# shiyao-li/NextBestPath

Hardware: AMD Instinct MI355X
Metric: exploration steps/s (+ NBP maps/s) at 256x256 (higher is better)
Workload: dtype f32

## Files before the change

### nextbestpath_amd/csrc/nbp_sim.hip

```cpp
#include "common.h"
#include "nbp_carve.h"
#include "nbp_camera.h"
#pragma clang fp contract(off)

namespace {

__device__ __forceinline__ void shade_pixel(const float* __restrict__ verts, const int* __restrict__ faces,
                                            const float* __restrict__ vcolors, const Cam& cam, int fi, int row, int col, int H,
                                            int W, float tanh_fov, float ambient, float* rgb3) {
    float v[3][3];
    const int i0 = faces[3 * (size_t)fi], i1 = faces[3 * (size_t)fi + 1], i2 = faces[3 * (size_t)fi + 2];
    to_view(verts + 3 * (size_t)i0, cam.R, cam.T, v[0]);
    to_view(verts + 3 * (size_t)i1, cam.R, cam.T, v[1]);
    to_view(verts + 3 * (size_t)i2, cam.R, cam.T, v[2]);
    float e1[3], e2[3], q[3];
#pragma unroll
    for (int c = 0; c < 3; ++c) { e1[c] = v[1][c] - v[0][c]; e2[c] = v[2][c] - v[0][c]; }
    q[0] = e1[1] * v[0][2] - e1[2] * v[0][1];
    q[1] = e1[2] * v[0][0] - e1[0] * v[0][2];
    q[2] = e1[0] * v[0][1] - e1[1] * v[0][0];
    const int s = H < W ? H : W;
    const float dx = pixel_centre_ndc(W, s, col) * tanh_fov;
    const float dy = pixel_centre_ndc(H, s, row) * tanh_fov;
    const float a0 = e1[2] * e2[1] - e1[1] * e2[2], a1 = e1[0] * e2[2] - e1[2] * e2[0], a2 = e1[1] * e2[0] - e1[0] * e2[1];
    const float u0 = v[0][1] * e2[2] - v[0][2] * e2[1], u1 = v[0][2] * e2[0] - v[0][0] * e2[2], u2 = v[0][0] * e2[1] - v[0][1] * e2[0];
    const float inv = 1.f / ((a0 * dx + a1 * dy) + a2);
    const float u = ((u0 * dx + u1 * dy) + u2) * inv;
    const float vv = ((dx * q[0] + dy * q[1]) + q[2]) * inv;
    const float w0 = (1.f - u) - vv;
    const float* c0 = vcolors + 3 * (size_t)i0;
    const float* c1 = vcolors + 3 * (size_t)i1;
    const float* c2 = vcolors + 3 * (size_t)i2;
#pragma unroll
    for (int k = 0; k < 3; ++k) rgb3[k] = ambient * ((w0 * c0[k] + u * c1[k]) + vv * c2[k]);
}


constexpr int COMPACT_CHUNK = 2048;

__device__ __forceinline__ bool pixel_valid(const float* d, const unsigned char* mk, int p, float fov_range) {
    const float z = d[p];
    return (mk ? mk[p] != 0 : z > -1.f) && z < fov_range;
}

__global__ __launch_bounds__(256) void unproject_count_kernel(const float* __restrict__ depth,
                                                              const unsigned char* __restrict__ mask, int HW, int nblk,
                                                              float fov_range, int* __restrict__ blk_count) {
    __shared__ int tot;
    const int f = blockIdx.y, b = blockIdx.x;
    const float* d = depth + (size_t)f * HW;
    const unsigned char* mk = mask ? mask + (size_t)f * HW : nullptr;
    if (threadIdx.x == 0) tot = 0;
    __syncthreads();
    int c = 0;
    for (int p = b * COMPACT_CHUNK + threadIdx.x; p < min((b + 1) * COMPACT_CHUNK, HW); p += 256)
// ... 232 lines not shown
}
__global__ __launch_bounds__(256) void unproject_compact4_kernel(const float* __restrict__ depth, const unsigned char* __restrict__ mask,
                                                                 int HW, int nblk, float fov_range, double gather,
                                                                 const int* __restrict__ blk_count, unsigned* __restrict__ list,
                                                                 int* __restrict__ counts) {
    unproject_compact4_body(blockIdx.x, blockIdx.y, gridDim.x, gridDim.y, depth, mask, HW, nblk, fov_range, gather, blk_count, list, counts);
}
__global__ __launch_bounds__(256) void unproject_compact4_batch_kernel(UnprojBatch b, int HW, int nblk, float fov_range, double gather) {
    const UnprojItem& a = b.it[blockIdx.z];
    unproject_compact4_body(blockIdx.x, blockIdx.y, gridDim.x, gridDim.y, a.depth[blockIdx.y] - (size_t)blockIdx.y * HW, nullptr, HW, nblk,
                            fov_range, gather, a.blk_count, b.list(blockIdx.z), a.counts);
}
template <bool COLOUR>
__global__ __launch_bounds__(256) void unproject_append_kernel(const float* __restrict__ depth, CamSet cams, int H, int W, float tanh_fov,
                                                               unsigned seed, const unsigned* __restrict__ list,
                                                               const int* __restrict__ counts, float* __restrict__ cloud,
                                                               long long* __restrict__ cloud_count, long long capacity, int n_frames,
                                                               int* __restrict__ done_ticket, const float* __restrict__ rgb,
                                                               float* __restrict__ cloud_rgb, const unsigned long long* __restrict__ zface,
                                                               const float* __restrict__ verts, const int* __restrict__ faces,
                                                               const float* __restrict__ vcolors, float ambient, int fence, BinFile bf) {
    unproject_append_body<COLOUR>(blockIdx.x, blockIdx.y, gridDim.x, gridDim.y, depth, cams.c, H, W, tanh_fov, seed, list, counts, cloud, cloud_count,
                          capacity, n_frames, done_ticket, rgb, cloud_rgb, zface, verts, faces, vcolors, ambient, fence, bf);
}
template <bool COLOUR>
__global__ __launch_bounds__(256) void unproject_append_batch_kernel(UnprojBatch b, int H, int W, float tanh_fov, int n_frames, float ambient,
                                                                     int fence) {
    const UnprojItem& a = b.it[blockIdx.z];
    const size_t shift = (size_t)blockIdx.y * H * W;
    unproject_append_body<COLOUR>(blockIdx.x, blockIdx.y, gridDim.x, gridDim.y, a.depth[blockIdx.y] - shift, a.cam, H, W, tanh_fov, a.seed,
                          b.list(blockIdx.z), a.counts, a.cloud, a.cloud_count, a.capacity, n_frames, b.ticket(blockIdx.z), nullptr, a.cloud_rgb,
                          a.zface[blockIdx.y] ? a.zface[blockIdx.y] - shift : nullptr, a.verts, a.faces, a.vcolors, ambient, fence);
}

__global__ void cloud_count_update_kernel(const int* __restrict__ counts, int F, long long* __restrict__ cloud_count,
                                          long long capacity) {
    if (blockIdx.x == 0 && threadIdx.x == 0) {
        long long n = *cloud_count;
        for (int f = 0; f < F; ++f) n += counts[2 * f + 1];
        *cloud_count = n < capacity ? n : capacity;
    }
}

constexpr int TILE = 8;
struct FaceRec { float a[3], un[3], q[3], tnum, pad[2]; };

constexpr int COARSE = 8;
constexpr int SEG_DEFAULT = 16384;
constexpr int HITS = 320;
constexpr unsigned ZBUF_EMPTY = 0x7F7F7F7Fu;

struct BinEntry { int face; unsigned box; };

__device__ __forceinline__ void raster_setup_body(unsigned bx, unsigned by, unsigned gx, unsigned gy, const float* __restrict__ verts, const int* __restrict__ faces,
                                                           int n_faces, const Cam* cams, int H, int W,
                                                           float tanh_fov, float zclip, FaceRec* __restrict__ recs,
                                                           int ctiles_x, int ctiles_y, int* __restrict__ ccount,
                                                           BinEntry* __restrict__ clist, unsigned* __restrict__ zbuf_bits,
                                                           unsigned long long* __restrict__ zface) {
    const int fr = by;
    const int fi = bx * blockDim.x + threadIdx.x;
    if (zface) for (int p = fi; p < H * W; p += gx * blockDim.x) zface[(size_t)fr * H * W + p] = ~0ull;
    else for (int p = fi; p < H * W; p += gx * blockDim.x) zbuf_bits[(size_t)fr * H * W + p] = ZBUF_EMPTY;
    bool have = false;
    int tx0 = 0, tx1 = 0, ty0 = 0, ty1 = 0;
    if (fi < n_faces) {
        const Cam cam = cams[fr];
        float v[3][3];
#pragma unroll
        for (int k = 0; k < 3; ++k) to_view(verts + 3 * (size_t)faces[3 * (size_t)fi + k], cam.R, cam.T, v[k]);
        if (!(v[0][2] <= zclip && v[1][2] <= zclip && v[2][2] <= zclip)) {
            FaceRec r;
            float e1[3], e2[3];
            const float* v0 = v[0];
#pragma unroll
            for (int c = 0; c < 3; ++c) { e1[c] = v[1][c] - v[0][c]; e2[c] = v[2][c] - v[0][c]; }
            r.q[0] = e1[1] * v0[2] - e1[2] * v0[1];
            r.q[1] = e1[2] * v0[0] - e1[0] * v0[2];
            r.q[2] = e1[0] * v0[1] - e1[1] * v0[0];
            r.tnum = (e2[0] * r.q[0] + e2[1] * r.q[1]) + e2[2] * r.q[2];
            r.a[0] = e1[2] * e2[1] - e1[1] * e2[2]; r.a[1] = e1[0] * e2[2] - e1[2] * e2[0]; r.a[2] = e1[1] * e2[0] - e1[0] * e2[1];
            r.un[0] = v0[1] * e2[2] - v0[2] * e2[1]; r.un[1] = v0[2] * e2[0] - v0[0] * e2[2]; r.un[2] = v0[0] * e2[1] - v0[1] * e2[0];
            r.pad[0] = r.pad[1] = 0.f;
            const int s = H < W ? H : W;
            float cmin = 1e30f, cmax = -1e30f, rmin = 1e30f, rmax = -1e30f;
            auto emit = [&](float x, float y, float z) {
                const float nx = x / (z * tanh_fov), ny = y / (z * tanh_fov);
                const float col = ((float)W - (float)s * nx - 1.f) * 0.5f;
                const float row = ((float)H - (float)s * ny - 1.f) * 0.5f;
                cmin = fminf(cmin, col); cmax = fmaxf(cmax, col); rmin = fminf(rmin, row); rmax = fmaxf(rmax, row);
            };
#pragma unroll
            for (int k = 0; k < 3; ++k) {
                const float* a = v[k];
                const float* b = v[(k + 1) % 3];
                const bool ain = a[2] >= zclip, bin_ = b[2] >= zclip;
                if (ain) emit(a[0], a[1], a[2]);
                if (ain != bin_) {
                    const float t = (zclip - a[2]) / (b[2] - a[2]);
                    emit(a[0] + t * (b[0] - a[0]), a[1] + t * (b[1] - a[1]), zclip);
                }
            }
            if (cmax >= cmin) {
                int c0 = (int)floorf(fmaxf(cmin, -1e8f)) - 1, c1 = (int)ceilf(fminf(cmax, 1e8f)) + 1;
                int r0 = (int)floorf(fmaxf(rmin, -1e8f)) - 1, r1 = (int)ceilf(fminf(rmax, 1e8f)) + 1;
                c0 = max(c0, 0); r0 = max(r0, 0); c1 = min(c1, W - 1); r1 = min(r1, H - 1);
                if (c0 <= c1 && r0 <= r1) {
                    recs[(size_t)fr * n_faces + fi] = r;
                    have = true;
                    tx0 = c0 / TILE; tx1 = c1 / TILE; ty0 = r0 / TILE; ty1 = r1 / TILE;
                }
            }
        }
    }
    const int lane = threadIdx.x & 63;
    const unsigned long long lt = (1ull << lane) - 1ull;
    const BinEntry e = {fi, (unsigned)tx0 | ((unsigned)tx1 << 8) | ((unsigned)ty0 << 16) | ((unsigned)ty1 << 24)};
    const int nct = ctiles_x * ctiles_y;
    for (int c0 = 0; c0 < nct; c0 += 64) {
        const int npass = min(64, nct - c0);
        int my_cnt = 0;
        for (int c = 0; c < npass; ++c) {
            const int cx = (c0 + c) % ctiles_x, cy = (c0 + c) / ctiles_x;
            const bool hit = have && tx0 <= cx * COARSE + COARSE - 1 && tx1 >= cx * COARSE && ty0 <= cy * COARSE + COARSE - 1 &&
                             ty1 >= cy * COARSE;
            const int n = __popcll(__ballot(hit));
            if (lane == c) my_cnt = n;
        }
        int my_base = 0;
        if (my_cnt > 0) my_base = atomicAdd(&ccount[fr * nct + c0 + lane], my_cnt);
        for (int c = 0; c < npass; ++c) {
            const int cx = (c0 + c) % ctiles_x, cy = (c0 + c) / ctiles_x;
            const bool hit = have && tx0 <= cx * COARSE + COARSE - 1 && tx1 >= cx * COARSE && ty0 <= cy * COARSE + COARSE - 1 &&
                             ty1 >= cy * COARSE;
            const unsigned long long bal = __ballot(hit);
            const int base = __shfl(my_base, c);
            if (hit) clist[((size_t)fr * nct + c0 + c) * n_faces + base + __popcll(bal & lt)] = e;
        }
    }
}

constexpr int RB = 2;
__device__ __forceinline__ int ballot_rank(unsigned long long bal) {
    return (int)__builtin_amdgcn_mbcnt_hi((unsigned)(bal >> 32), __builtin_amdgcn_mbcnt_lo((unsigned)bal, 0u));
}
__device__ __forceinline__ void raster_block_body(unsigned bx, unsigned by, const FaceRec* __restrict__ recs, int n_faces, int H, int W,
                                                  float tanh_fov, float zclip, int tiles_x, int tiles_y, int ctiles_x,
                                                  const int* __restrict__ ccount, const BinEntry* __restrict__ clist,
                                                  unsigned* __restrict__ zbuf_bits, unsigned long long* __restrict__ zface, int SEG) {
    __shared__ BinEntry bhits[HITS];
    __shared__ int nb_sh;
    __shared__ __attribute__((aligned(16))) FaceRec sh[4][64];
    __shared__ int shf[4][64];
    const int fr = by;
    const int blocks_x = (tiles_x + RB - 1) / RB, blocks_y = (tiles_y + RB - 1) / RB;
    const int nblocks = blocks_x * blocks_y;
    const int blk = bx % nblocks, seg = bx / nblocks;
    const int bxx = blk % blocks_x, byy = blk / blocks_x;
    const int nct = ctiles_x * ((tiles_y + COARSE - 1) / COARSE);
    const int ct = ((byy * RB) / COARSE) * ctiles_x + (bxx * RB) / COARSE;
    const int n = ccount[fr * nct + ct];
    const int s0 = seg * SEG;
    if (s0 >= n) return;
    const int s1 = min(n, s0 + SEG);
    const int tid = threadIdx.x, lane = tid & 63, wave = __builtin_amdgcn_readfirstlane(tid >> 6);
    const BinEntry* lst = clist + ((size_t)fr * nct + ct) * n_faces;
    const int btx0 = bxx * RB, btx1 = btx0 + RB - 1, bty0 = byy * RB, bty1 = bty0 + RB - 1;
    const int tx = btx0 + (wave & 1), ty = bty0 + (wave >> 1);
    const bool live = tx < tiles_x && ty < tiles_y;
    const int col = tx * TILE + (lane & 7), row = ty * TILE + (lane >> 3);
    const int s = H < W ? H : W;
    const float ndc_x = pixel_centre_ndc(W, s, col);
    const float ndc_y = pixel_centre_ndc(H, s, row);
    const float dx = ndc_x * tanh_fov, dy = ndc_y * tanh_fov;
    const FaceRec* rb = recs + (size_t)fr * n_faces;
    float zbest = 3.0e38f;
    int fbest = -1;
    const float eps = 1e-6f;
    for (int c0 = s0; c0 < s1; c0 += HITS) {
        const int c1 = min(s1, c0 + HITS);
        if (tid == 0) nb_sh = 0;
        __syncthreads();
        for (int base = c0; base < c1; base += 256) {
            bool in = false;
            BinEntry e = {0, 0u};
            if (base + tid < c1) {
                e = lst[base + tid];
                in = btx1 >= (int)(e.box & 255u) && btx0 <= (int)((e.box >> 8) & 255u) && bty1 >= (int)((e.box >> 16) & 255u) &&
                     bty0 <= (int)(e.box >> 24);
            }
            const unsigned long long bal = __ballot(in);
            int wbase = 0;
            if (lane == 0 && bal) wbase = atomicAdd(&nb_sh, __popcll(bal));
            wbase = __shfl(wbase, 0);
            if (in) bhits[wbase + ballot_rank(bal)] = e;
        }
        __syncthreads();
        const int nb = nb_sh;
        if (live)
            for (int hb = 0; hb < nb; hb += 64) {
                bool in = false;
                int face = 0;
                if (hb + lane < nb) {
                    const BinEntry e = bhits[hb + lane];
                    face = e.face;
                    in = tx >= (int)(e.box & 255u) && tx <= (int)((e.box >> 8) & 255u) && ty >= (int)((e.box >> 16) & 255u) &&
                         ty <= (int)(e.box >> 24);
                }
                const unsigned long long bal = __ballot(in);
                const int m = __popcll(bal);
                if (in) {
                    const int k = ballot_rank(bal);
                    sh[wave][k] = rb[face];
                    shf[wave][k] = face;
                }
                __builtin_amdgcn_s_waitcnt(0);
                __builtin_amdgcn_wave_barrier();
                for (int k = 0; k < m; ++k) {
                    const FaceRec& f = sh[wave][k];
                    const float det = (f.a[0] * dx + f.a[1] * dy) + f.a[2];
                    if (fabsf(det) < 1e-12f) continue;
                    const float inv = 1.f / det;
                    const float u = ((f.un[0] * dx + f.un[1] * dy) + f.un[2]) * inv;
                    const float vv = ((dx * f.q[0] + dy * f.q[1]) + f.q[2]) * inv;
                    const float z = f.tnum * inv;
                    if (u >= -eps && vv >= -eps && u + vv <= 1.f + eps && z > zclip) {
                        const int fid = shf[wave][k];
                        if (z < zbest || (z == zbest && fid < fbest)) { zbest = z; fbest = fid; }
                    }
                }
                __builtin_amdgcn_wave_barrier();
            }
        __syncthreads();
    }
    if (live && row < H && col < W && zbest < 1.0e38f) {
        const size_t pix = ((size_t)fr * H + row) * W + col;
        if (zface) atomicMin(&zface[pix], ((unsigned long long)__float_as_uint(zbest) << 32) | (unsigned)fbest);
        else atomicMin(&zbuf_bits[pix], __float_as_uint(zbest));
    }
}

__global__ __launch_bounds__(256) void raster_finalize_kernel(float* __restrict__ zbuf, long long n) {
    for (long long i = (long long)blockIdx.x * blockDim.x + threadIdx.x; i < n; i += (long long)gridDim.x * blockDim.x)
        if (!(zbuf[i] < 1.0e38f)) zbuf[i] = -1.f;
}

__device__ __forceinline__ void raster_shade_body(unsigned bx, unsigned by, unsigned gx, unsigned gy, const unsigned long long* __restrict__ zface,
                                                           const float* __restrict__ verts, const int* __restrict__ faces,
                                                           const float* __restrict__ vcolors, const Cam* cams, int H, int W,
                                                           float tanh_fov, float ambient, float* __restrict__ zbuf_or_null,
                                                           float* __restrict__ rgb_or_null, double* __restrict__ gray_sum) {
    const int fr = by;
    const int p = bx * blockDim.x + threadIdx.x;
    float gray = 0.f;
    if (p < H * W) {
        const size_t pix = (size_t)fr * H * W + p;
        const unsigned long long zf = zface[pix];
        float c[3] = {1.f, 1.f, 1.f};
        if (zbuf_or_null) zbuf_or_null[pix] = zf != ~0ull ? __uint_as_float((unsigned)(zf >> 32)) : -1.f;
        if (rgb_or_null) {
            if (zf != ~0ull) shade_pixel(verts, faces, vcolors, cams[fr], (int)(unsigned)zf, p / W, p % W, H, W, tanh_fov, ambient, c);
            rgb_or_null[3 * pix] = c[0]; rgb_or_null[3 * pix + 1] = c[1]; rgb_or_null[3 * pix + 2] = c[2];
            gray = (0.299f * c[0] + 0.587f * c[1]) + 0.114f * c[2];
        }
    }
    if (!gray_sum) return;
    double gs = (double)gray;
    for (int o = 32; o; o >>= 1) gs += __shfl_xor(gs, o);
    if ((threadIdx.x & 63) == 0) atomicAdd(&gray_sum[fr], gs);
}

struct RasterItem {
    const float* verts; const int* faces; const float* vcolors; FaceRec* recs; int* ccount; BinEntry* clist; float* zbuf;
    unsigned long long* zface; int n_faces; unsigned gx_setup, gx_tile; Cam cam[4];
};
struct RasterBatch { RasterItem it[STEP_BATCH]; };

__global__ __launch_bounds__(256) void raster_setup_kernel(const float* __restrict__ verts, const int* __restrict__ faces, int n_faces,
                                                           CamSet cams, int H, int W, float tanh_fov, float zclip,
                                                           FaceRec* __restrict__ recs, int ctiles_x, int ctiles_y, int* __restrict__ ccount,
                                                           BinEntry* __restrict__ clist, unsigned* __restrict__ zbuf_bits,
                                                           unsigned long long* __restrict__ zface) {
    raster_setup_body(blockIdx.x, blockIdx.y, gridDim.x, gridDim.y, verts, faces, n_faces, cams.c, H, W, tanh_fov, zclip, recs, ctiles_x,
                      ctiles_y, ccount, clist, zbuf_bits, zface);
}
__global__ __launch_bounds__(256) void raster_clear_batch_kernel(RasterBatch b, int n_counters) {
    int* c = b.it[blockIdx.y].ccount;
    for (int i = blockIdx.x * blockDim.x + threadIdx.x; i < n_counters; i += gridDim.x * blockDim.x) c[i] = 0;
}
__global__ __launch_bounds__(256) void raster_setup_batch_kernel(RasterBatch b, int H, int W, float tanh_fov, float zclip, int ctiles_x,
                                                                 int ctiles_y) {
    const RasterItem& a = b.it[blockIdx.z];
    if (blockIdx.x >= a.gx_setup) return;
    raster_setup_body(blockIdx.x, blockIdx.y, a.gx_setup, gridDim.y, a.verts, a.faces, a.n_faces, a.cam, H, W, tanh_fov, zclip, a.recs,
                      ctiles_x, ctiles_y, a.ccount, a.clist, nullptr, a.zface);
}
__global__ __launch_bounds__(256) void raster_tile_kernel(const FaceRec* __restrict__ recs, int n_faces, int H, int W, float tanh_fov,
                                                          float zclip, int tiles_x, int tiles_y, int ctiles_x, int ctiles_y,
                                                          const int* __restrict__ ccount, const BinEntry* __restrict__ clist,
                                                          unsigned* __restrict__ zbuf_bits, unsigned long long* __restrict__ zface, int SEG) {
    raster_block_body(blockIdx.x, blockIdx.y, recs, n_faces, H, W, tanh_fov, zclip, tiles_x, tiles_y, ctiles_x, ccount, clist, zbuf_bits, zface,
                      SEG);
}
__global__ __launch_bounds__(256) void raster_tile_batch_kernel(RasterBatch b, int H, int W, float tanh_fov, float zclip, int tiles_x,
                                                                int tiles_y, int ctiles_x, int ctiles_y, int SEG) {
    const RasterItem& a = b.it[blockIdx.z];
    if (blockIdx.x >= a.gx_tile) return;
    raster_block_body(blockIdx.x, blockIdx.y, a.recs, a.n_faces, H, W, tanh_fov, zclip, tiles_x, tiles_y, ctiles_x, a.ccount, a.clist, nullptr,
                      a.zface, SEG);
}
__global__ __launch_bounds__(256) void raster_shade_kernel(const unsigned long long* __restrict__ zface, const float* __restrict__ verts,
                                                           const int* __restrict__ faces, const float* __restrict__ vcolors, CamSet cams,
                                                           int H, int W, float tanh_fov, float ambient, float* __restrict__ zbuf_or_null,
                                                           float* __restrict__ rgb_or_null, double* __restrict__ gray_sum) {
    raster_shade_body(blockIdx.x, blockIdx.y, gridDim.x, gridDim.y, zface, verts, faces, vcolors, cams.c, H, W, tanh_fov, ambient, zbuf_or_null,
                      rgb_or_null, gray_sum);
}
__global__ __launch_bounds__(256) void raster_depth_batch_kernel(RasterBatch b, int H, int W, float tanh_fov) {
    const RasterItem& a = b.it[blockIdx.z];
    raster_shade_body(blockIdx.x, blockIdx.y, gridDim.x, gridDim.y, a.zface, a.verts, a.faces, a.vcolors, a.cam, H, W, tanh_fov, 0.f, a.zbuf,
                      nullptr, nullptr);
}

__global__ __launch_bounds__(256) void contrast_kernel(float* __restrict__ rgb, int HW3, const double* __restrict__ gray_sum,
                                                       int HW, float factor) {
    const int fr = blockIdx.y;
    const float mean = (float)(gray_sum[fr] / (double)HW);
    for (int i = blockIdx.x * blockDim.x + threadIdx.x; i < HW3; i += gridDim.x * blockDim.x) {
        const float v = factor * rgb[(size_t)fr * HW3 + i] + (1.f - factor) * mean;
        rgb[(size_t)fr * HW3 + i] = fminf(fmaxf(v, 0.f), 1.f);
    }
}

__device__ __forceinline__ float ray_tri(const float* o, const float* d, const float* a, const float* b, const float* c) {
    const float e1[3] = {b[0] - a[0], b[1] - a[1], b[2] - a[2]};
    const float e2[3] = {c[0] - a[0], c[1] - a[1], c[2] - a[2]};
    const float p[3] = {d[1] * e2[2] - d[2] * e2[1], d[2] * e2[0] - d[0] * e2[2], d[0] * e2[1] - d[1] * e2[0]};
    const float det = (e1[0] * p[0] + e1[1] * p[1]) + e1[2] * p[2];
    if (fabsf(det) < 1e-12f) return -1.f;
    const float inv = 1.f / det;
    const float tv[3] = {o[0] - a[0], o[1] - a[1], o[2] - a[2]};
    const float u = ((tv[0] * p[0] + tv[1] * p[1]) + tv[2] * p[2]) * inv;
    if (u < 0.f || u > 1.f) return -1.f;
    const float q[3] = {tv[1] * e1[2] - tv[2] * e1[1], tv[2] * e1[0] - tv[0] * e1[2], tv[0] * e1[1] - tv[1] * e1[0]};
    const float v = ((d[0] * q[0] + d[1] * q[1]) + d[2] * q[2]) * inv;
    if (v < 0.f || u + v > 1.f) return -1.f;
    const float t = ((e2[0] * q[0] + e2[1] * q[1]) + e2[2] * q[2]) * inv;
    return t > 0.f ? t : -1.f;
}

__global__ __launch_bounds__(256) void segments_hit_kernel(const float* __restrict__ verts, const int* __restrict__ faces,
                                                           int n_faces, const float* __restrict__ segs, int* __restrict__ hit) {
    const int e = blockIdx.y;
    const int fi = blockIdx.x * blockDim.x + threadIdx.x;
    if (fi >= n_faces) return;
    const float* sg = segs + 6 * (size_t)e;
    float d[3] = {sg[3] - sg[0], sg[4] - sg[1], sg[5] - sg[2]};
    const float len = sqrtf((d[0] * d[0] + d[1] * d[1]) + d[2] * d[2]);
    if (!(len > 0.f)) return;
    d[0] /= len; d[1] /= len; d[2] /= len;
    const int* f = faces + 3 * (size_t)fi;
    const float t = ray_tri(sg, d, verts + 3 * (size_t)f[0], verts + 3 * (size_t)f[1], verts + 3 * (size_t)f[2]);
// ... 280 lines not shown
                                                 list, counts2);
    if ((rc = nbp_launch_status())) return rc;
    auto append = cloud_rgb_or_null ? unproject_append_kernel<true> : unproject_append_kernel<false>;
    append<<<grid, 256, 0, st>>>(depth, cams, H, W, tan_half_fov, seed, list, counts2, cloud, cloud_count, capacity, n_frames, nullptr,
                                 rgb_or_null, cloud_rgb_or_null, sh.zface, sh.verts, sh.faces, sh.vcolors, sh.ambient, 0,
                                 BinFile{nullptr, nullptr, nullptr, 0});
    if ((rc = nbp_launch_status())) return rc;
    cloud_count_update_kernel<<<1, 64, 0, st>>>(counts2, n_frames, cloud_count, capacity);
    return nbp_launch_status();
}

constexpr size_t RASTER_WS_SLACK = 256;
struct RasterWs { FaceRec* recs; int* ccount; BinEntry* clist; unsigned long long* zface; double* gray; size_t nct; };
static RasterWs raster_ws_layout(Carver& c, int n_faces, int n_frames, int H, int W, bool rgb) {
    const size_t nct = (size_t)nbp_cdiv(nbp_cdiv(W, TILE), COARSE) * nbp_cdiv(nbp_cdiv(H, TILE), COARSE) * n_frames;
    return {c.take<FaceRec>((size_t)n_frames * n_faces), c.take<int>(nct), c.take<BinEntry>(nct * n_faces),
            rgb ? c.take<unsigned long long>((size_t)n_frames * H * W) : nullptr, rgb ? c.take<double>(MAX_CAMS) : nullptr, nct};
}
static size_t raster_ws_bytes(int n_faces, int n_frames, int H, int W, bool rgb) {
    if (n_faces < 1 || n_frames < 1 || H < 1 || W < 1) return 0;
    return carved_bytes(RASTER_WS_SLACK, raster_ws_layout, n_faces, n_frames, H, W, rgb);
}

extern "C" size_t nbp_raster_workspace_bytes(int n_faces, int n_frames, int H, int W, int bin_cap) {
    (void)bin_cap;
    return raster_ws_bytes(n_faces, n_frames, H, W, false);
}

extern "C" size_t nbp_raster_rgb_workspace_bytes(int n_faces, int n_frames, int H, int W) {
    return raster_ws_bytes(n_faces, n_frames, H, W, true);
}

static int raster_launch(const float* verts, int n_verts, const int* faces, int n_faces, const float* cams12_host, int n_frames,
                         int H, int W, float tan_half_fov, float z_clip, float* zbuf, const float* vcolors, float ambient,
                         float contrast, float* rgb, void* ws, size_t ws_bytes, void* stream,
                         unsigned long long* zface_out = nullptr) {
    NBP_RETURN_IF(!verts || !faces || !cams12_host || !zbuf || !ws, NBP_E_ARG);
    NBP_RETURN_IF(n_verts < 3 || n_faces < 1 || n_frames < 1 || n_frames > MAX_CAMS || H < 1 || W < 1, NBP_E_ARG);
    NBP_RETURN_IF(!(z_clip > 0.f), NBP_E_ARG);
    const int tiles_x = (int)nbp_cdiv(W, TILE), tiles_y = (int)nbp_cdiv(H, TILE);
    NBP_RETURN_IF(tiles_x > 256 || tiles_y > 256, NBP_E_SHAPE);
    NBP_RETURN_IF(ws_bytes < raster_ws_bytes(n_faces, n_frames, H, W, rgb != nullptr && !zface_out), NBP_E_WS);
    hipStream_t st = (hipStream_t)stream;
    const int ctiles_x = (int)nbp_cdiv(tiles_x, COARSE), ctiles_y = (int)nbp_cdiv(tiles_y, COARSE);
    const RasterWs L = carve(ws, raster_ws_layout, n_faces, n_frames, H, W, rgb != nullptr && !zface_out);
    FaceRec* const recs = L.recs;
    int* const ccount = L.ccount;
    BinEntry* const clist = L.clist;
    unsigned long long* const zface = zface_out ? zface_out : L.zface;
    double* const gray = L.gray;
    const long long npx = (long long)n_frames * H * W;
    hipError_t e = hipMemsetAsync(ccount, 0, L.nct * sizeof(int), st);
    if (e != hipSuccess) return (int)e;
    dim3 g1((unsigned)nbp_cdiv(n_faces, 256), (unsigned)n_frames);
    raster_setup_kernel<<<g1, 256, 0, st>>>(verts, faces, n_faces, camset_from_host(cams12_host, n_frames), H, W,
                                            tan_half_fov, z_clip, recs, ctiles_x, ctiles_y, ccount, clist, (unsigned*)zbuf, zface);
    int rc = nbp_launch_status();
    if (rc) return rc;
    const bool need_gray = gray && contrast != 1.f;
    if (need_gray) {
        e = hipMemsetAsync(gray, 0, (size_t)n_frames * sizeof(double), st);
        if (e != hipSuccess) return (int)e;
    }
    constexpr int SEG = SEG_DEFAULT;
    const int nseg = (int)nbp_cdiv(n_faces, SEG);
    dim3 g2((unsigned)((int)nbp_cdiv(tiles_x, RB) * (int)nbp_cdiv(tiles_y, RB) * nseg), (unsigned)n_frames);
    raster_tile_kernel<<<g2, 256, 0, st>>>(recs, n_faces, H, W, tan_half_fov, z_clip, tiles_x, tiles_y, ctiles_x, ctiles_y,
                                          ccount, clist, (unsigned*)zbuf, zface, SEG);
    if ((rc = nbp_launch_status())) return rc;
    if (!zface) {
        raster_finalize_kernel<<<nbp_ew_grid(npx, 256), 256, 0, st>>>(zbuf, npx);
        return nbp_launch_status();
    }
    dim3 g3((unsigned)nbp_cdiv((long long)H * W, 256), (unsigned)n_frames);
    raster_shade_kernel<<<g3, 256, 0, st>>>(zface, verts, faces, vcolors, camset_from_host(cams12_host, n_frames), H, W,
                                            tan_half_fov, ambient, zbuf, rgb, need_gray ? gray : nullptr);
    if ((rc = nbp_launch_status())) return rc;
    if (need_gray) {
        dim3 g4((unsigned)nbp_ew_grid((long long)H * W * 3, 256), (unsigned)n_frames);
        contrast_kernel<<<g4, 256, 0, st>>>(rgb, H * W * 3, gray, H * W, contrast);
        rc = nbp_launch_status();
    }
    return rc;
}

extern "C" int nbp_raster_zbuf_f32(const float* verts, int n_verts, const int* faces, int n_faces, const float* cams12_host,
                                   int n_frames, int H, int W, float tan_half_fov, float z_clip, int bin_cap, float* zbuf,
                                   int* overflow_flag, void* ws, size_t ws_bytes, void* stream) {
    NBP_ENTER();
    (void)bin_cap; (void)overflow_flag;
    return raster_launch(verts, n_verts, faces, n_faces, cams12_host, n_frames, H, W, tan_half_fov, z_clip, zbuf, nullptr, 0.f,
                         1.f, nullptr, ws, ws_bytes, stream);
}

extern "C" int nbp_raster_rgbz_f32(const float* verts, int n_verts, const int* faces, int n_faces, const float* vcolors3,
                                   const float* cams12_host, int n_frames, int H, int W, float tan_half_fov, float z_clip,
                                   float ambient, float contrast_factor, float* zbuf, float* rgb, void* ws, size_t ws_bytes,
                                   void* stream) {
    NBP_ENTER();
    NBP_RETURN_IF(!vcolors3 || !rgb, NBP_E_ARG);
    return raster_launch(verts, n_verts, faces, n_faces, cams12_host, n_frames, H, W, tan_half_fov, z_clip, zbuf, vcolors3,
                         ambient, contrast_factor, rgb, ws, ws_bytes, stream);
}

extern "C" int nbp_raster_zface_f32(const float* verts, int n_verts, const int* faces, int n_faces, const float* cams12_host,
                                    int n_frames, int H, int W, float tan_half_fov, float z_clip, float* zbuf, void* zface,
                                    void* ws, size_t ws_bytes, void* stream) {
    NBP_ENTER();
    NBP_RETURN_IF(!zface, NBP_E_ARG);
    return raster_launch(verts, n_verts, faces, n_faces, cams12_host, n_frames, H, W, tan_half_fov, z_clip, zbuf, nullptr, 0.f,
                         1.f, nullptr, ws, ws_bytes, stream, (unsigned long long*)zface);
}

extern "C" int nbp_unproject_append_shaded_batch_f32(int n, const float* const* depth, const void* const* zface, const float* const* verts,
                                                     const int* const* faces, const float* const* vcolors, const float* cams12_host,
                                                     int n_frames, int H, int W, float tan_half_fov, float fov_range,
                                                     double gathering_factor, const unsigned* seeds, float ambient, int* const* counts2,
                                                     float* const* cloud, float* const* cloud_rgb, long long* const* cloud_count,
                                                     const long long* capacity, void* const* ws, size_t ws_bytes_each, void* stream) {
    NBP_ENTER();
    NBP_RETURN_IF(n < 1 || n > STEP_BATCH || !depth || !cams12_host || !seeds || !counts2 || !cloud || !cloud_count || !capacity || !ws, NBP_E_ARG);
    NBP_RETURN_IF(n_frames < 1 || n_frames > 4 || H < 2 || W < 2 || !(gathering_factor >= 0.0 && gathering_factor <= 1.0), NBP_E_ARG);
    NBP_RETURN_IF(ws_bytes_each < nbp_unproject_workspace_bytes(n_frames, H, W), NBP_E_WS);
    const int HW = H * W;
    NBP_RETURN_IF((HW & 3) != 0, NBP_E_SHAPE);
// ... 3 lines not shown
    UnprojBatch b;
    bool any_colour = false;
    for (int r = 0; r < STEP_BATCH; ++r) {
        const int q = r < n ? r : 0;
        NBP_RETURN_IF(!counts2[q] || !cloud[q] || !cloud_count[q] || capacity[q] < 1 || !ws[q], NBP_E_ARG);
        UnprojItem& a = b.it[r];
        const UnprojectWs L = carve(ws[q], unproject_ws_layout, n_frames, H, W);
        a.blk_count = L.blk_count;
        b.ticket_off = (int)(L.ticket - L.blk_count);
        b.list_off_bytes = (unsigned)((char*)L.list - (char*)L.blk_count);
        a.counts = counts2[q]; a.cloud = cloud[q]; a.cloud_count = cloud_count[q]; a.capacity = capacity[q];
        const bool col = zface && zface[(size_t)q * n_frames] && cloud_rgb && cloud_rgb[q] && verts && faces && vcolors;
        a.cloud_rgb = col ? cloud_rgb[q] : nullptr;
        any_colour = any_colour || col;
        for (int f = 0; f < 4; ++f) {
            const int g = f < n_frames ? f : 0;
            a.depth[f] = depth[(size_t)q * n_frames + g];
            NBP_RETURN_IF(!a.depth[f] || ((uintptr_t)a.depth[f] & 15) != 0, NBP_E_ARG);
            a.zface[f] = col ? (const unsigned long long*)zface[(size_t)q * n_frames + g] : nullptr;
        }
        a.verts = col ? verts[q] : nullptr; a.faces = col ? faces[q] : nullptr; a.vcolors = col ? vcolors[q] : nullptr;
        a.seed = seeds[q];
        cams_from_host(cams12_host + (size_t)q * n_frames * 12, n_frames, a.cam, 4);
    }
    dim3 g4((unsigned)nb4, (unsigned)n_frames, (unsigned)n);
    unproject_count4_batch_kernel<<<g4, 256, 0, st>>>(b, HW, nb4, fov_range);
    int rc = nbp_launch_status();
    if (rc) return rc;
    unproject_compact4_batch_kernel<<<g4, 256, 0, st>>>(b, HW, nb4, fov_range, gathering_factor);
    if ((rc = nbp_launch_status())) return rc;
    const int max_keep = (int)((double)H * W * gathering_factor) + 1;
    dim3 grid((unsigned)nbp_cdiv(max_keep, 256), (unsigned)n_frames, (unsigned)n);
    auto append = any_colour ? unproject_append_batch_kernel<true> : unproject_append_batch_kernel<false>;
    append<<<grid, 256, 0, st>>>(b, H, W, tan_half_fov, n_frames, ambient, ticket_fence());
    return nbp_launch_status();
}

extern "C" int nbp_raster_zface_batch_f32(int n, const float* const* verts, const int* n_verts, const int* const* faces, const int* n_faces,
                                          const float* cams12_host, int n_frames, int H, int W, float tan_half_fov, float z_clip,
                                          float* const* zbuf, void* const* zface, void* const* ws, const size_t* ws_bytes, void* stream) {
    NBP_ENTER();
    NBP_RETURN_IF(n < 1 || n > STEP_BATCH || !verts || !n_verts || !faces || !n_faces || !cams12_host || !zbuf || !zface || !ws || !ws_bytes,
                  NBP_E_ARG);
    NBP_RETURN_IF(n_frames < 1 || n_frames > 4 || H < 1 || W < 1, NBP_E_ARG);
    NBP_RETURN_IF(!(z_clip > 0.f), NBP_E_ARG);
    const int tiles_x = (int)nbp_cdiv(W, TILE), tiles_y = (int)nbp_cdiv(H, TILE);
    NBP_RETURN_IF(tiles_x > 256 || tiles_y > 256, NBP_E_SHAPE);
    hipStream_t st = (hipStream_t)stream;
    const int ctiles_x = (int)nbp_cdiv(tiles_x, COARSE), ctiles_y = (int)nbp_cdiv(tiles_y, COARSE);
    const size_t nct = (size_t)ctiles_x * ctiles_y * n_frames;
    constexpr int SEG = SEG_DEFAULT;
    RasterBatch b;
    unsigned g_setup = 1, g_tile = 1;
    for (int r = 0; r < STEP_BATCH; ++r) {
        const int q = r < n ? r : 0;
        NBP_RETURN_IF(!verts[q] || !faces[q] || n_verts[q] < 3 || n_faces[q] < 1 || !zbuf[q] || !zface[q] || !ws[q], NBP_E_ARG);
        NBP_RETURN_IF(ws_bytes[q] < raster_ws_bytes(n_faces[q], n_frames, H, W, false), NBP_E_WS);
        RasterItem& a = b.it[r];
        const RasterWs L = carve(ws[q], raster_ws_layout, n_faces[q], n_frames, H, W, false);
        a.recs = L.recs; a.ccount = L.ccount; a.clist = L.clist;
        a.verts = verts[q]; a.faces = faces[q]; a.vcolors = nullptr; a.zbuf = zbuf[q]; a.zface = (unsigned long long*)zface[q];
        a.n_faces = n_faces[q];
        a.gx_setup = r < n ? (unsigned)nbp_cdiv(n_faces[q], 256) : 0;
        a.gx_tile = r < n ? (unsigned)((int)nbp_cdiv(tiles_x, RB) * (int)nbp_cdiv(tiles_y, RB) * (int)nbp_cdiv(n_faces[q], SEG)) : 0;
        if (a.gx_setup > g_setup) g_setup = a.gx_setup;
        if (a.gx_tile > g_tile) g_tile = a.gx_tile;
        cams_from_host(cams12_host + (size_t)q * n_frames * 12, n_frames, a.cam, 4);
    }
    raster_clear_batch_kernel<<<dim3(1, (unsigned)n), 256, 0, st>>>(b, (int)nct);
    int rc = nbp_launch_status();
    if (rc) return rc;
    raster_setup_batch_kernel<<<dim3(g_setup, (unsigned)n_frames, (unsigned)n), 256, 0, st>>>(b, H, W, tan_half_fov, z_clip, ctiles_x, ctiles_y);
    if ((rc = nbp_launch_status())) return rc;
    raster_tile_batch_kernel<<<dim3(g_tile, (unsigned)n_frames, (unsigned)n), 256, 0, st>>>(b, H, W, tan_half_fov, z_clip, tiles_x, tiles_y,
                                                                                          ctiles_x, ctiles_y, SEG);
    if ((rc = nbp_launch_status())) return rc;
    raster_depth_batch_kernel<<<dim3((unsigned)nbp_cdiv((long long)H * W, 256), (unsigned)n_frames, (unsigned)n), 256, 0, st>>>(b, H, W,
                                                                                                                          tan_half_fov);
    return nbp_launch_status();
}

extern "C" int nbp_shade_image_f32(const void* zface, const float* verts, const int* faces, const float* vcolors3,
                                   const float* cams12_host, int n_frames, int H, int W, float tan_half_fov, float ambient,
                                   float contrast_factor, float* rgb, void* stream) {
    NBP_ENTER();
    NBP_RETURN_IF(!zface || !verts || !faces || !vcolors3 || !cams12_host || !rgb, NBP_E_ARG);
    NBP_RETURN_IF(n_frames < 1 || n_frames > MAX_CAMS || H < 1 || W < 1, NBP_E_ARG);
    NBP_RETURN_IF(contrast_factor != 1.f, NBP_E_SHAPE);
    dim3 g3((unsigned)nbp_cdiv((long long)H * W, 256), (unsigned)n_frames);
    raster_shade_kernel<<<g3, 256, 0, (hipStream_t)stream>>>((const unsigned long long*)zface, verts, faces, vcolors3,
                                                             camset_from_host(cams12_host, n_frames), H, W, tan_half_fov,
                                                             ambient, nullptr, rgb, nullptr);
    return nbp_launch_status();
}

extern "C" int nbp_segments_hit_mesh_f32(const float* verts, const int* faces, int n_faces, const float* segs6, int n_segs,
                                         int* hit, void* stream) {
    NBP_ENTER();
    NBP_RETURN_IF(!verts || !faces || !segs6 || !hit || n_faces < 1 || n_segs < 1 || n_segs > 65535, NBP_E_ARG);
    hipStream_t st = (hipStream_t)stream;
    hipError_t e = hipMemsetAsync(hit, 0, (size_t)n_segs * sizeof(int), st);
    if (e != hipSuccess) return (int)e;
    dim3 g((unsigned)nbp_cdiv(n_faces, 256), (unsigned)n_segs);
    segments_hit_kernel<<<g, 256, 0, st>>>(verts, faces, n_faces, segs6, hit);
    return nbp_launch_status();
}

extern "C" int nbp_axis_ray_counts_f32(const float* verts, const int* faces, int n_faces, const float* pts3, int n_pts,
                                       int* counts3, void* stream) {
    NBP_ENTER();
    NBP_RETURN_IF(!verts || !faces || !pts3 || !counts3 || n_faces < 1 || n_pts < 1 || n_pts > 65535, NBP_E_ARG);
    hipStream_t st = (hipStream_t)stream;
    hipError_t e = hipMemsetAsync(counts3, 0, (size_t)n_pts * 3 * sizeof(int), st);
    if (e != hipSuccess) return (int)e;
    dim3 g((unsigned)nbp_cdiv(n_faces, 256), (unsigned)n_pts);
    axis_ray_count_kernel<<<g, 256, 0, st>>>(verts, faces, n_faces, pts3, counts3);
    return nbp_launch_status();
}

extern "C" int nbp_carve_update_f32(const float* proxy_pts3, int P, const float* depth, const unsigned char* mask_or_null,
                                    const float* cam12_host, int H, int W, float tan_half_fov, float zfar, float fov_range,
                                    float tol, float score_threshold, float* n_inside, float* n_behind, float* occ,
                                    float* out_of_field, void* stream) {
    NBP_ENTER();
    NBP_RETURN_IF(!proxy_pts3 || !depth || !cam12_host || !n_inside || !n_behind || !occ || !out_of_field, NBP_E_ARG);
    NBP_RETURN_IF(P < 1 || H < 2 || W < 2, NBP_E_ARG);
    Cam cam;
    for (int k = 0; k < 9; ++k) cam.R[k] = cam12_host[k];
    for (int k = 0; k < 3; ++k) cam.T[k] = cam12_host[9 + k];
// ... 234 lines not shown
```

Before: 2369.

## Add conservative tile-level face culling and owner-writes path for single-segment rasterization

Adds a conservative interval test that rejects faces which cannot cover any pixel of an 8x8 tile before the per-pixel ray-triangle loop. When the face count fits in one segment, each tile block now owns its pixels: it writes depth and face id directly instead of pre-clearing the buffers, using atomicMin, and running the separate depth/finalize pass. Binning now walks only the wave's bounding rectangle of coarse tiles instead of every coarse tile. Together these cut clears, atomics, a kernel launch and wasted intersection work, at the cost of extra per-face cull arithmetic and more template code paths.

Result: no change. 2389, median of 4 (+0.8%).

```diff
diff --git a/nextbestpath_amd/csrc/nbp_raster_cull.h b/nextbestpath_amd/csrc/nbp_raster_cull.h
--- /dev/null
+++ b/nextbestpath_amd/csrc/nbp_raster_cull.h
@@ -0,0 +1,52 @@
+#pragma once
+#include <math.h>
+
+#if defined(__HIPCC__)
+#define NBP_CULL_HD __host__ __device__ __forceinline__
+#else
+#define NBP_CULL_HD inline
+#endif
+#if defined(__clang__)
+#pragma clang fp contract(off)
+#endif
+#if defined(__HIP_DEVICE_COMPILE__)
+#define NBP_CULL_PHASE() __builtin_amdgcn_sched_barrier(0)
+#else
+#define NBP_CULL_PHASE() ((void)0)
+#endif
+
+constexpr float RASTER_CULL_H8 = 4.76837158203125e-7f;
+constexpr float RASTER_CULL_TINY = 1e-30f;
+constexpr float RASTER_CULL_EPS = 2e-6f;
+
+struct RasterCullRange { float lo, hi, err; };
+
+NBP_CULL_HD RasterCullRange raster_cull_range(float c0, float c1, float c2, float s, float dxa, float dxb, float dya, float dyb) {
+    const float mx = fmaxf(fabsf(dxa), fabsf(dxb)), my = fmaxf(fabsf(dya), fabsf(dyb));
+    const float xa = c0 * dxa, xb = c0 * dxb, ya = c1 * dya, yb = c1 * dyb;
+    const float l0 = s * ((xa + ya) + c2), l1 = s * ((xb + ya) + c2), l2 = s * ((xa + yb) + c2), l3 = s * ((xb + yb) + c2);
+    RasterCullRange r;
+    r.lo = fminf(fminf(l0, l1), fminf(l2, l3));
+    r.hi = fmaxf(fmaxf(l0, l1), fmaxf(l2, l3));
+    r.err = RASTER_CULL_H8 * ((fabsf(c0) * mx + fabsf(c1) * my) + fabsf(c2)) + RASTER_CULL_TINY;
+    return r;
+}
+
+NBP_CULL_HD bool raster_cull_reject(const float* a, const float* un, const float* q, float tnum, float dxa, float dxb, float dya,
+                                    float dyb) {
+    const float s = (a[0] * dxa + a[1] * dya) + a[2] > 0.f ? 1.f : -1.f;
+    const RasterCullRange D = raster_cull_range(a[0], a[1], a[2], s, dxa, dxb, dya, dyb);
+    if (!(D.lo > 2.f * D.err)) return false;
+    if (s * tnum <= 0.f) return true;
+    const float dm = D.hi + 2.f * D.err;
+    NBP_CULL_PHASE();
+    const RasterCullRange U = raster_cull_range(un[0], un[1], un[2], s, dxa, dxb, dya, dyb);
+    if (U.hi < -(RASTER_CULL_EPS * dm + 2.f * U.err)) return true;
+    NBP_CULL_PHASE();
+    const RasterCullRange Q = raster_cull_range(q[0], q[1], q[2], s, dxa, dxb, dya, dyb);
+    if (Q.hi < -(RASTER_CULL_EPS * dm + 2.f * Q.err)) return true;
+    const float lim = (dm + RASTER_CULL_EPS * dm) + 4.f * (U.err + Q.err);
+    NBP_CULL_PHASE();
+    const RasterCullRange W = raster_cull_range(un[0] + q[0], un[1] + q[1], un[2] + q[2], s, dxa, dxb, dya, dyb);
+    return W.lo > lim && W.hi <= 3.0e38f;
+}
diff --git a/nextbestpath_amd/csrc/nbp_sim.hip b/nextbestpath_amd/csrc/nbp_sim.hip
--- a/nextbestpath_amd/csrc/nbp_sim.hip
+++ b/nextbestpath_amd/csrc/nbp_sim.hip
@@ -1,6 +1,7 @@
 #include "common.h"
 #include "nbp_carve.h"
 #include "nbp_camera.h"
+#include "nbp_raster_cull.h"
 #pragma clang fp contract(off)
 
 namespace {
@@ -339,6 +340,7 @@
 
 struct BinEntry { int face; unsigned box; };
 
+template <bool OWN>
 __device__ __forceinline__ void raster_setup_body(unsigned bx, unsigned by, unsigned gx, unsigned gy, const float* __restrict__ verts, const int* __restrict__ faces,
                                                            int n_faces, const Cam* cams, int H, int W,
                                                            float tanh_fov, float zclip, FaceRec* __restrict__ recs,
@@ -347,8 +349,10 @@
                                                            unsigned long long* __restrict__ zface) {
     const int fr = by;
     const int fi = bx * blockDim.x + threadIdx.x;
-    if (zface) for (int p = fi; p < H * W; p += gx * blockDim.x) zface[(size_t)fr * H * W + p] = ~0ull;
-    else for (int p = fi; p < H * W; p += gx * blockDim.x) zbuf_bits[(size_t)fr * H * W + p] = ZBUF_EMPTY;
+    if (!OWN) {
+        if (zface) for (int p = fi; p < H * W; p += gx * blockDim.x) zface[(size_t)fr * H * W + p] = ~0ull;
+        else for (int p = fi; p < H * W; p += gx * blockDim.x) zbuf_bits[(size_t)fr * H * W + p] = ZBUF_EMPTY;
+    }
     bool have = false;
     int tx0 = 0, tx1 = 0, ty0 = 0, ty1 = 0;
     if (fi < n_faces) {
@@ -404,25 +408,37 @@
     const unsigned long long lt = (1ull << lane) - 1ull;
     const BinEntry e = {fi, (unsigned)tx0 | ((unsigned)tx1 << 8) | ((unsigned)ty0 << 16) | ((unsigned)ty1 << 24)};
     const int nct = ctiles_x * ctiles_y;
-    for (int c0 = 0; c0 < nct; c0 += 64) {
-        const int npass = min(64, nct - c0);
+    int rx0 = have ? tx0 / COARSE : 0x7fff, rx1 = have ? tx1 / COARSE : -1, ry0 = have ? ty0 / COARSE : 0x7fff, ry1 = have ? ty1 / COARSE : -1;
+    for (int o = 32; o; o >>= 1) {
+        rx0 = min(rx0, __shfl_xor(rx0, o)); rx1 = max(rx1, __shfl_xor(rx1, o));
+        ry0 = min(ry0, __shfl_xor(ry0, o)); ry1 = max(ry1, __shfl_xor(ry1, o));
+    }
+    rx0 = __builtin_amdgcn_readfirstlane(rx0); rx1 = __builtin_amdgcn_readfirstlane(rx1);
+    ry0 = __builtin_amdgcn_readfirstlane(ry0); ry1 = __builtin_amdgcn_readfirstlane(ry1);
+    if (rx1 < rx0) return;
+    const int rw = rx1 - rx0 + 1, nrect = rw * (ry1 - ry0 + 1);
+    for (int c0 = 0; c0 < nrect; c0 += 64) {
+        const int npass = min(64, nrect - c0);
         int my_cnt = 0;
         for (int c = 0; c < npass; ++c) {
-            const int cx = (c0 + c) % ctiles_x, cy = (c0 + c) / ctiles_x;
+            const int cx = rx0 + (c0 + c) % rw, cy = ry0 + (c0 + c) / rw;
             const bool hit = have && tx0 <= cx * COARSE + COARSE - 1 && tx1 >= cx * COARSE && ty0 <= cy * COARSE + COARSE - 1 &&
                              ty1 >= cy * COARSE;
             const int n = __popcll(__ballot(hit));
             if (lane == c) my_cnt = n;
         }
         int my_base = 0;
-        if (my_cnt > 0) my_base = atomicAdd(&ccount[fr * nct + c0 + lane], my_cnt);
+        if (my_cnt > 0) {
+            const int i = c0 + lane;
+            my_base = atomicAdd(&ccount[fr * nct + (ry0 + i / rw) * ctiles_x + rx0 + i % rw], my_cnt);
+        }
         for (int c = 0; c < npass; ++c) {
-            const int cx = (c0 + c) % ctiles_x, cy = (c0 + c) / ctiles_x;
+            const int cx = rx0 + (c0 + c) % rw, cy = ry0 + (c0 + c) / rw;
             const bool hit = have && tx0 <= cx * COARSE + COARSE - 1 && tx1 >= cx * COARSE && ty0 <= cy * COARSE + COARSE - 1 &&
                              ty1 >= cy * COARSE;
             const unsigned long long bal = __ballot(hit);
             const int base = __shfl(my_base, c);
-            if (hit) clist[((size_t)fr * nct + c0 + c) * n_faces + base + __popcll(bal & lt)] = e;
+            if (hit) clist[((size_t)fr * nct + cy * ctiles_x + cx) * n_faces + base + __popcll(bal & lt)] = e;
         }
     }
 }
@@ -431,6 +447,7 @@
 __device__ __forceinline__ int ballot_rank(unsigned long long bal) {
     return (int)__builtin_amdgcn_mbcnt_hi((unsigned)(bal >> 32), __builtin_amdgcn_mbcnt_lo((unsigned)bal, 0u));
 }
+template <bool OWN>
 __device__ __forceinline__ void raster_block_body(unsigned bx, unsigned by, const FaceRec* __restrict__ recs, int n_faces, int H, int W,
                                                   float tanh_fov, float zclip, int tiles_x, int tiles_y, int ctiles_x,
                                                   const int* __restrict__ ccount, const BinEntry* __restrict__ clist,
@@ -448,7 +465,7 @@
     const int ct = ((byy * RB) / COARSE) * ctiles_x + (bxx * RB) / COARSE;
     const int n = ccount[fr * nct + ct];
     const int s0 = seg * SEG;
-    if (s0 >= n) return;
+    if (!OWN && s0 >= n) return;
     const int s1 = min(n, s0 + SEG);
     const int tid = threadIdx.x, lane = tid & 63, wave = __builtin_amdgcn_readfirstlane(tid >> 6);
     const BinEntry* lst = clist + ((size_t)fr * nct + ct) * n_faces;
@@ -460,6 +477,10 @@
     const float ndc_x = pixel_centre_ndc(W, s, col);
     const float ndc_y = pixel_centre_ndc(H, s, row);
     const float dx = ndc_x * tanh_fov, dy = ndc_y * tanh_fov;
+    const float dxa = __int_as_float(__builtin_amdgcn_readlane(__float_as_int(dx), 0));
+    const float dxb = __int_as_float(__builtin_amdgcn_readlane(__float_as_int(dx), 7));
+    const float dya = __int_as_float(__builtin_amdgcn_readlane(__float_as_int(dy), 0));
+    const float dyb = __int_as_float(__builtin_amdgcn_readlane(__float_as_int(dy), 56));
     const FaceRec* rb = recs + (size_t)fr * n_faces;
     float zbest = 3.0e38f;
     int fbest = -1;
@@ -498,12 +519,22 @@
                 const int m = __popcll(bal);
                 if (in) {
                     const int k = ballot_rank(bal);
-                    sh[wave][k] = rb[face];
+                    const FaceRec& r = rb[face];
+                    FaceRec& d = sh[wave][k];
+#pragma unroll
+                    for (int c = 0; c < 3; ++c) { d.a[c] = r.a[c]; d.un[c] = r.un[c]; d.q[c] = r.q[c]; }
+                    d.tnum = r.tnum;
                     shf[wave][k] = face;
                 }
                 __builtin_amdgcn_s_waitcnt(0);
                 __builtin_amdgcn_wave_barrier();
-                for (int k = 0; k < m; ++k) {
+                bool keep = false;
+                if (lane < m) {
+                    const FaceRec& f = sh[wave][lane];
+                    keep = !raster_cull_reject(f.a, f.un, f.q, f.tnum, dxa, dxb, dya, dyb);
+                }
+                for (unsigned long long todo = __ballot(keep); todo; todo &= todo - 1ull) {
+                    const int k = __builtin_ctzll(todo);
                     const FaceRec& f = sh[wave][k];
                     const float det = (f.a[0] * dx + f.a[1] * dy) + f.a[2];
                     if (fabsf(det) < 1e-12f) continue;
@@ -520,7 +551,14 @@
             }
         __syncthreads();
     }
-    if (live && row < H && col < W && zbest < 1.0e38f) {
+    if (OWN) {
+        if (live && row < H && col < W) {
+            const size_t pix = ((size_t)fr * H + row) * W + col;
+            const bool hit = zbest < 1.0e38f;
+            if (zface) zface[pix] = hit ? ((unsigned long long)__float_as_uint(zbest) << 32) | (unsigned)fbest : ~0ull;
+            if (zbuf_bits) zbuf_bits[pix] = __float_as_uint(hit ? zbest : -1.f);
+        }
+    } else if (live && row < H && col < W && zbest < 1.0e38f) {
         const size_t pix = ((size_t)fr * H + row) * W + col;
         if (zface) atomicMin(&zface[pix], ((unsigned long long)__float_as_uint(zbest) << 32) | (unsigned)fbest);
         else atomicMin(&zbuf_bits[pix], __float_as_uint(zbest));
@@ -563,38 +601,42 @@
 };
 struct RasterBatch { RasterItem it[STEP_BATCH]; };
 
+template <bool OWN>
 __global__ __launch_bounds__(256) void raster_setup_kernel(const float* __restrict__ verts, const int* __restrict__ faces, int n_faces,
                                                            CamSet cams, int H, int W, float tanh_fov, float zclip,
                                                            FaceRec* __restrict__ recs, int ctiles_x, int ctiles_y, int* __restrict__ ccount,
                                                            BinEntry* __restrict__ clist, unsigned* __restrict__ zbuf_bits,
                                                            unsigned long long* __restrict__ zface) {
-    raster_setup_body(blockIdx.x, blockIdx.y, gridDim.x, gridDim.y, verts, faces, n_faces, cams.c, H, W, tanh_fov, zclip, recs, ctiles_x,
+    raster_setup_body<OWN>(blockIdx.x, blockIdx.y, gridDim.x, gridDim.y, verts, faces, n_faces, cams.c, H, W, tanh_fov, zclip, recs, ctiles_x,
                       ctiles_y, ccount, clist, zbuf_bits, zface);
 }
 __global__ __launch_bounds__(256) void raster_clear_batch_kernel(RasterBatch b, int n_counters) {
     int* c = b.it[blockIdx.y].ccount;
     for (int i = blockIdx.x * blockDim.x + threadIdx.x; i < n_counters; i += gridDim.x * blockDim.x) c[i] = 0;
 }
+template <bool OWN>
 __global__ __launch_bounds__(256) void raster_setup_batch_kernel(RasterBatch b, int H, int W, float tanh_fov, float zclip, int ctiles_x,
                                                                  int ctiles_y) {
     const RasterItem& a = b.it[blockIdx.z];
     if (blockIdx.x >= a.gx_setup) return;
-    raster_setup_body(blockIdx.x, blockIdx.y, a.gx_setup, gridDim.y, a.verts, a.faces, a.n_faces, a.cam, H, W, tanh_fov, zclip, a.recs,
+    raster_setup_body<OWN>(blockIdx.x, blockIdx.y, a.gx_setup, gridDim.y, a.verts, a.faces, a.n_faces, a.cam, H, W, tanh_fov, zclip, a.recs,
                       ctiles_x, ctiles_y, a.ccount, a.clist, nullptr, a.zface);
 }
+template <bool OWN>
 __global__ __launch_bounds__(256) void raster_tile_kernel(const FaceRec* __restrict__ recs, int n_faces, int H, int W, float tanh_fov,
                                                           float zclip, int tiles_x, int tiles_y, int ctiles_x, int ctiles_y,
                                                           const int* __restrict__ ccount, const BinEntry* __restrict__ clist,
                                                           unsigned* __restrict__ zbuf_bits, unsigned long long* __restrict__ zface, int SEG) {
-    raster_block_body(blockIdx.x, blockIdx.y, recs, n_faces, H, W, tanh_fov, zclip, tiles_x, tiles_y, ctiles_x, ccount, clist, zbuf_bits, zface,
-                      SEG);
-}
+    raster_block_body<OWN>(blockIdx.x, blockIdx.y, recs, n_faces, H, W, tanh_fov, zclip, tiles_x, tiles_y, ctiles_x, ccount, clist, zbuf_bits,
+                           zface, SEG);
+}
+template <bool OWN>
 __global__ __launch_bounds__(256) void raster_tile_batch_kernel(RasterBatch b, int H, int W, float tanh_fov, float zclip, int tiles_x,
                                                                 int tiles_y, int ctiles_x, int ctiles_y, int SEG) {
     const RasterItem& a = b.it[blockIdx.z];
     if (blockIdx.x >= a.gx_tile) return;
-    raster_block_body(blockIdx.x, blockIdx.y, a.recs, a.n_faces, H, W, tanh_fov, zclip, tiles_x, tiles_y, ctiles_x, a.ccount, a.clist, nullptr,
-                      a.zface, SEG);
+    raster_block_body<OWN>(blockIdx.x, blockIdx.y, a.recs, a.n_faces, H, W, tanh_fov, zclip, tiles_x, tiles_y, ctiles_x, a.ccount, a.clist,
+                           OWN ? (unsigned*)a.zbuf : nullptr, a.zface, SEG);
 }
 __global__ __launch_bounds__(256) void raster_shade_kernel(const unsigned long long* __restrict__ zface, const float* __restrict__ verts,
                                                            const int* __restrict__ faces, const float* __restrict__ vcolors, CamSet cams,
@@ -981,9 +1023,13 @@
     const long long npx = (long long)n_frames * H * W;
     hipError_t e = hipMemsetAsync(ccount, 0, L.nct * sizeof(int), st);
     if (e != hipSuccess) return (int)e;
+    constexpr int SEG = SEG_DEFAULT;
+    const int nseg = (int)nbp_cdiv(n_faces, SEG);
+    const bool own = nseg == 1;
     dim3 g1((unsigned)nbp_cdiv(n_faces, 256), (unsigned)n_frames);
-    raster_setup_kernel<<<g1, 256, 0, st>>>(verts, faces, n_faces, camset_from_host(cams12_host, n_frames), H, W,
-                                            tan_half_fov, z_clip, recs, ctiles_x, ctiles_y, ccount, clist, (unsigned*)zbuf, zface);
+    (own ? raster_setup_kernel<true> : raster_setup_kernel<false>)<<<g1, 256, 0, st>>>(
+        verts, faces, n_faces, camset_from_host(cams12_host, n_frames), H, W, tan_half_fov, z_clip, recs, ctiles_x, ctiles_y, ccount, clist,
+        (unsigned*)zbuf, zface);
     int rc = nbp_launch_status();
     if (rc) return rc;
     const bool need_gray = gray && contrast != 1.f;
@@ -991,15 +1037,19 @@
         e = hipMemsetAsync(gray, 0, (size_t)n_frames * sizeof(double), st);
         if (e != hipSuccess) return (int)e;
     }
-    constexpr int SEG = SEG_DEFAULT;
-    const int nseg = (int)nbp_cdiv(n_faces, SEG);
     dim3 g2((unsigned)((int)nbp_cdiv(tiles_x, RB) * (int)nbp_cdiv(tiles_y, RB) * nseg), (unsigned)n_frames);
-    raster_tile_kernel<<<g2, 256, 0, st>>>(recs, n_faces, H, W, tan_half_fov, z_clip, tiles_x, tiles_y, ctiles_x, ctiles_y,
-                                          ccount, clist, (unsigned*)zbuf, zface, SEG);
-    if ((rc = nbp_launch_status())) return rc;
-    if (!zface) {
-        raster_finalize_kernel<<<nbp_ew_grid(npx, 256), 256, 0, st>>>(zbuf, npx);
-        return nbp_launch_status();
+    if (own) {
+        raster_tile_kernel<true><<<g2, 256, 0, st>>>(recs, n_faces, H, W, tan_half_fov, z_clip, tiles_x, tiles_y, ctiles_x, ctiles_y, ccount,
+                                                     clist, rgb ? nullptr : (unsigned*)zbuf, zface, SEG);
+        if ((rc = nbp_launch_status()) || !rgb) return rc;
+    } else {
+        raster_tile_kernel<false><<<g2, 256, 0, st>>>(recs, n_faces, H, W, tan_half_fov, z_clip, tiles_x, tiles_y, ctiles_x, ctiles_y, ccount,
+                                                      clist, (unsigned*)zbuf, zface, SEG);
+        if ((rc = nbp_launch_status())) return rc;
+        if (!zface) {
+            raster_finalize_kernel<<<nbp_ew_grid(npx, 256), 256, 0, st>>>(zbuf, npx);
+            return nbp_launch_status();
+        }
     }
     dim3 g3((unsigned)nbp_cdiv((long long)H * W, 256), (unsigned)n_frames);
     raster_shade_kernel<<<g3, 256, 0, st>>>(zface, verts, faces, vcolors, camset_from_host(cams12_host, n_frames), H, W,
@@ -1109,6 +1159,7 @@
     constexpr int SEG = SEG_DEFAULT;
     RasterBatch b;
     unsigned g_setup = 1, g_tile = 1;
+    bool own = true;
     for (int r = 0; r < STEP_BATCH; ++r) {
         const int q = r < n ? r : 0;
         NBP_RETURN_IF(!verts[q] || !faces[q] || n_verts[q] < 3 || n_faces[q] < 1 || !zbuf[q] || !zface[q] || !ws[q], NBP_E_ARG);
@@ -1120,6 +1171,7 @@
         a.n_faces = n_faces[q];
         a.gx_setup = r < n ? (unsigned)nbp_cdiv(n_faces[q], 256) : 0;
         a.gx_tile = r < n ? (unsigned)((int)nbp_cdiv(tiles_x, RB) * (int)nbp_cdiv(tiles_y, RB) * (int)nbp_cdiv(n_faces[q], SEG)) : 0;
+        own = own && nbp_cdiv(n_faces[q], SEG) == 1;
         if (a.gx_setup > g_setup) g_setup = a.gx_setup;
         if (a.gx_tile > g_tile) g_tile = a.gx_tile;
         cams_from_host(cams12_host + (size_t)q * n_frames * 12, n_frames, a.cam, 4);
@@ -1127,11 +1179,12 @@
     raster_clear_batch_kernel<<<dim3(1, (unsigned)n), 256, 0, st>>>(b, (int)nct);
     int rc = nbp_launch_status();
     if (rc) return rc;
-    raster_setup_batch_kernel<<<dim3(g_setup, (unsigned)n_frames, (unsigned)n), 256, 0, st>>>(b, H, W, tan_half_fov, z_clip, ctiles_x, ctiles_y);
+    (own ? raster_setup_batch_kernel<true> : raster_setup_batch_kernel<false>)<<<dim3(g_setup, (unsigned)n_frames, (unsigned)n), 256, 0, st>>>(
+        b, H, W, tan_half_fov, z_clip, ctiles_x, ctiles_y);
     if ((rc = nbp_launch_status())) return rc;
-    raster_tile_batch_kernel<<<dim3(g_tile, (unsigned)n_frames, (unsigned)n), 256, 0, st>>>(b, H, W, tan_half_fov, z_clip, tiles_x, tiles_y,
-                                                                                          ctiles_x, ctiles_y, SEG);
-    if ((rc = nbp_launch_status())) return rc;
+    (own ? raster_tile_batch_kernel<true> : raster_tile_batch_kernel<false>)<<<dim3(g_tile, (unsigned)n_frames, (unsigned)n), 256, 0, st>>>(
+        b, H, W, tan_half_fov, z_clip, tiles_x, tiles_y, ctiles_x, ctiles_y, SEG);
+    if ((rc = nbp_launch_status()) || own) return rc;
     raster_depth_batch_kernel<<<dim3((unsigned)nbp_cdiv((long long)H * W, 256), (unsigned)n_frames, (unsigned)n), 256, 0, st>>>(b, H, W,
                                                                                                                           tan_half_fov);
     return nbp_launch_status();
```
